# refresh-bio/vclust

Hardware: AMD Instinct MI355X
Metric: genome pairs/sec through prefilter+align (ani.tsv) (higher is better)
Workload: dtype u64

## Files before the change

include/vclust_gpu.h:

```cpp
#ifndef VCLUST_GPU_H
#define VCLUST_GPU_H

#include <stdint.h>

#ifdef __cplusplus
extern "C" {
#endif

enum {
    VG_OK = 0, VG_EINVAL = -1, VG_EIO = -2, VG_ENODEV = -3, VG_EHIP = -4, VG_ENOMEM = -5,
    VG_EOVERFLOW = -6
};

const char* vg_version(void);
const char* vg_last_error(void);
void        vg_free(void* p);
int vg_device_count(void);
int vg_set_device(int device);
void vg_release_device_memory(void);
int vg_alloc_selftest(const int64_t* sizes, int n_sizes, int cycles);
int vg_copy(void* dst, const void* src, int64_t bytes, int to_host);

typedef struct vg_genomes vg_genomes;

// ... 4 lines not shown
int vg_genomes_from_codes(const uint8_t* codes, const int64_t* offsets, int n_genomes,
                          const char* const* names, vg_genomes** out);
void        vg_genomes_free(vg_genomes* g);
int         vg_genomes_count(const vg_genomes* g);
int64_t     vg_genomes_total_len(const vg_genomes* g);
int         vg_genomes_lengths(const vg_genomes* g, int64_t* out );
const char* vg_genomes_name(const vg_genomes* g, int idx);
int         vg_genomes_codes(const vg_genomes* g, int idx, uint8_t* out);
int vg_genomes_to_device(vg_genomes* g);

typedef struct { uint32_t a, b, shared; } vg_pair_count;

int vg_kmer_shared(vg_genomes* g, int k, double fraction, int shard, int n_shards,
                   uint32_t min_shared, int64_t* set_sizes, vg_pair_count** pairs,
                   int64_t* n_pairs);
int vg_kmer_shared_new(vg_genomes* g, int n_db, int k, double fraction, uint32_t min_shared, int64_t* set_sizes,
                       vg_pair_count** pairs, int64_t* n_pairs);
void vg_set_new_path(int mode);
typedef struct {
    int accepted; int64_t P; int n_passes;
    int levels, total_bits, B1, B2;
    int st_tiles; int64_t n_st; int u_st, g_st;
    int tile32k, narrow, short_rec;
} vg_kmer_geometry_info;
int vg_kmer_geometry(const vg_genomes* g, int k, double fraction, int shard, int n_shards, vg_kmer_geometry_info* info);
int vg_kmer_geometry_at(int64_t padded_positions, int k, vg_kmer_geometry_info* info);
int vg_kmer_set(vg_genomes* g, int idx, int k, double fraction, uint64_t** out, int64_t* n_out);

int vg_write_fltr(const vg_genomes* g, int k, double fraction, int min_kmers, double min_ident,
                  int max_seqs, const int64_t* set_sizes, const vg_pair_count* pairs,
                  int64_t n_pairs, const char* out_path);

int vg_filter_pairs(int k, int min_kmers, double min_ident, const int64_t* set_sizes, int64_t n_genomes,
                    const vg_pair_count* pairs, int64_t n_pairs, vg_pair_count** out, int64_t* n_out);

typedef struct {
    int    k;
    int    min_kmers;
    double min_ident;
    int    batch_size;
    double kmers_fraction;
    int    max_seqs;
    int    num_threads;
    int    verbosity;
    int    is_multifasta;
} vg_prefilter_params;
// ... 10 lines not shown
    uint32_t task; int32_t qstart, qend, rstart, rend; int32_t n_match;
} vg_region;

typedef struct { int weak_seed_ratio, anchor_margin, seed_choice; } vg_lz_fit;
void vg_set_lz_fit(const vg_lz_fit* f);

int vg_lz_align(vg_genomes* g, const vg_task* tasks, int64_t n_tasks, const vg_lz_params* p,
                vg_pair_stat* stats, vg_region** regions, int64_t* n_regions);

int vg_lz_prepare(vg_genomes* g, const vg_pair_count* pairs, int64_t n_pairs, const vg_lz_params* p);

int vg_align_order(const vg_genomes* g, int32_t* order );
int vg_read_filter(const vg_genomes* g, const char* path, double thr,
                   vg_pair_count** pairs, int64_t* n_pairs);

int vg_align_tasks(const vg_genomes* g, const vg_pair_count* pairs, int64_t n_pairs,
                   vg_task** tasks, int64_t* n_tasks);
int vg_lz_index_dump(vg_genomes* g, int idx, const vg_lz_params* p,
                     uint32_t** bucket_end, uint32_t** entries, int64_t* n_entries,
                     int* pos_bits, int* tag_bits, int* path);
void vg_set_index_budget(int64_t bytes);
void vg_set_subshards(int n);
void vg_set_range_scan(int mode);
void vg_set_placement_trials(int n);

typedef struct {
    vg_lz_params lz;
    double out_tani, out_gani, out_ani, out_qcov, out_rcov;
    const char* filter_path; double filter_threshold;
    const char* out_aln_path;
    const char* const* out_columns; int n_out_columns;
    int num_threads; int verbosity; int is_multifasta;
} vg_align_params;
int vg_write_ani(const vg_genomes* g, const vg_task* tasks, const vg_pair_stat* stats,
                 int64_t n_tasks, const vg_region* regions, int64_t n_regions,
                 const char* out_path, const vg_align_params* p);
int vg_align(const char* const* fasta_paths, int n_paths, const char* out_path,
             const vg_align_params* p);

int vg_align_new(const char* const* db_paths, int n_db_paths, const char* const* new_paths, int n_new_paths,
                 const char* out_path, const vg_align_params* p);

typedef struct vg_comm vg_comm;
typedef int (*vg_allgather_fn)(void* ctx, const void* send, void* recv, int64_t bytes, int on_device);
int  vg_comm_create(int rank, int world, vg_allgather_fn allgather, void* ctx, vg_comm** out);
int  vg_rccl_unique_id(void* out , int64_t bytes);
// ... 134 lines not shown
```

vclust_amd/_lib.py:

```python
import ctypes as C
import pathlib

PKG_DIR = pathlib.Path(__file__).resolve().parent
LIB_PATH = PKG_DIR / 'libvclust_gpu.so'


class VclustGpuError(RuntimeError):
    def __init__(self, code, msg):
        super().__init__(f'libvclust_gpu error {code}: {msg}')
        self.code = code


class PairCount(C.Structure):
    _fields_ = [('a', C.c_uint32), ('b', C.c_uint32), ('shared', C.c_uint32)]


class Task(C.Structure):
    _fields_ = [('q', C.c_uint32), ('r', C.c_uint32)]


class PairStat(C.Structure):
    _fields_ = [('n_match', C.c_uint32), ('aln_len', C.c_uint32), ('n_regions', C.c_uint32)]


# ... 53 lines not shown
class DedupStats(C.Structure):
    _fields_ = [('records', C.c_int64), ('unique', C.c_int64), ('removed', C.c_int64), ('reverse', C.c_int64),
                ('rounds', C.c_int64), ('collisions', C.c_int64)]


class DedupOptions(C.Structure):
    _fields_ = [('circular', C.c_int)]


class DedupContainedStats(C.Structure):
    _fields_ = [('passes', C.c_int64), ('positions', C.c_int64), ('hits', C.c_int64), ('candidates', C.c_int64),
                ('verified', C.c_int64), ('slices', C.c_int64)]


class DedupRepeatStats(C.Structure):
    _fields_ = [('with_repeat', C.c_int64), ('repeat_symbols', C.c_int64), ('candidates', C.c_int64), ('equal', C.c_int64),
                ('batches', C.c_int64)]


class KmerGeometry(C.Structure):
    _fields_ = [('accepted', C.c_int), ('P', C.c_int64), ('n_passes', C.c_int),
                ('levels', C.c_int), ('total_bits', C.c_int), ('B1', C.c_int), ('B2', C.c_int),
                ('st_tiles', C.c_int), ('n_st', C.c_int64), ('u_st', C.c_int), ('g_st', C.c_int),
                ('tile32k', C.c_int), ('narrow', C.c_int), ('short_rec', C.c_int)]


class KernelTime(C.Structure):
    _fields_ = [('name', C.c_char * 48), ('total_ms', C.c_double), ('launches', C.c_int64),
                ('bytes', C.c_double)]


ALLGATHER_FN = C.CFUNCTYPE(C.c_int, C.c_void_p, C.c_void_p, C.c_void_p, C.c_int64, C.c_int)

P = C.POINTER
SYMBOLS = {
    'vg_version': (C.c_char_p, []),
    'vg_last_error': (C.c_char_p, []),
    'vg_free': (None, [C.c_void_p]),
    'vg_device_count': (C.c_int, []),
    'vg_set_device': (C.c_int, [C.c_int]),
    'vg_release_device_memory': (None, []),
    'vg_copy': (C.c_int, [C.c_void_p, C.c_void_p, C.c_int64, C.c_int]),
    'vg_alloc_selftest': (C.c_int, [C.POINTER(C.c_int64), C.c_int, C.c_int]),
    'vg_genomes_load': (C.c_int, [P(C.c_char_p), C.c_int, C.c_int, C.c_int, P(C.c_void_p)]),
    'vg_genomes_load_db_new': (C.c_int, [P(C.c_char_p), C.c_int, P(C.c_char_p), C.c_int, C.c_int, C.c_int, P(C.c_void_p), P(C.c_int)]),
    'vg_genomes_from_codes': (C.c_int, [C.c_void_p, C.c_void_p, C.c_int, P(C.c_char_p), P(C.c_void_p)]),
    'vg_genomes_free': (None, [C.c_void_p]),
# ... 8 lines not shown
    'vg_kmer_shared_new': (C.c_int, [C.c_void_p, C.c_int, C.c_int, C.c_double, C.c_uint32, P(C.c_int64), P(P(PairCount)), P(C.c_int64)]),
    'vg_kmer_geometry': (C.c_int, [C.c_void_p, C.c_int, C.c_double, C.c_int, C.c_int, P(KmerGeometry)]),
    'vg_kmer_geometry_at': (C.c_int, [C.c_int64, C.c_int, P(KmerGeometry)]),
    'vg_kmer_set': (C.c_int, [C.c_void_p, C.c_int, C.c_int, C.c_double, P(P(C.c_uint64)), P(C.c_int64)]),
    'vg_filter_pairs': (C.c_int, [C.c_int, C.c_int, C.c_double, C.POINTER(C.c_int64), C.c_int64, C.POINTER(PairCount), C.c_int64,
                                  C.POINTER(C.POINTER(PairCount)), C.POINTER(C.c_int64)]),
    'vg_write_fltr': (C.c_int, [C.c_void_p, C.c_int, C.c_double, C.c_int, C.c_double, C.c_int,
                                P(C.c_int64), P(PairCount), C.c_int64, C.c_char_p]),
    'vg_prefilter': (C.c_int, [P(C.c_char_p), C.c_int, C.c_char_p, P(PrefilterParams)]),
    'vg_prefilter_new': (C.c_int, [P(C.c_char_p), C.c_int, P(C.c_char_p), C.c_int, C.c_char_p, P(PrefilterParams)]),
    'vg_set_process_ends_after_call': (None, [C.c_int]),
    'vg_set_lz_fit': (None, [P(LzFit)]),
    'vg_lz_align': (C.c_int, [C.c_void_p, P(Task), C.c_int64, P(LzParams), P(PairStat),
                              P(P(Region)), P(C.c_int64)]),
    'vg_align_order': (C.c_int, [C.c_void_p, P(C.c_int32)]),
    'vg_read_filter': (C.c_int, [C.c_void_p, C.c_char_p, C.c_double, P(P(PairCount)), P(C.c_int64)]),
    'vg_align_tasks': (C.c_int, [C.c_void_p, P(PairCount), C.c_int64, P(P(Task)), P(C.c_int64)]),
    'vg_lz_prepare': (C.c_int, [C.c_void_p, P(PairCount), C.c_int64, P(LzParams)]),
    'vg_lz_index_dump': (C.c_int, [C.c_void_p, C.c_int, P(LzParams), P(P(C.c_uint32)), P(P(C.c_uint32)), P(C.c_int64),
                                   P(C.c_int), P(C.c_int), P(C.c_int)]),
    'vg_set_index_budget': (None, [C.c_int64]),
    'vg_set_subshards': (None, [C.c_int]),
    'vg_set_range_scan': (None, [C.c_int]),
    'vg_set_new_path': (None, [C.c_int]),
    'vg_set_placement_trials': (None, [C.c_int]),
    'vg_write_ani': (C.c_int, [C.c_void_p, P(Task), P(PairStat), C.c_int64, P(Region), C.c_int64,
                               C.c_char_p, P(AlignParams)]),
    'vg_align': (C.c_int, [P(C.c_char_p), C.c_int, C.c_char_p, P(AlignParams)]),
    'vg_align_new': (C.c_int, [P(C.c_char_p), C.c_int, P(C.c_char_p), C.c_int, C.c_char_p, P(AlignParams)]),
    'vg_comm_create': (C.c_int, [C.c_int, C.c_int, C.c_void_p, C.c_void_p, P(C.c_void_p)]),
    'vg_rccl_unique_id': (C.c_int, [C.c_void_p, C.c_int64]),
    'vg_comm_rccl_create': (C.c_int, [C.c_int, C.c_int, C.c_void_p, C.c_int64, P(C.c_void_p)]),
    'vg_comm_free': (None, [C.c_void_p]),
    'vg_comm_kind': (C.c_int, [C.c_void_p]),
    'vg_comm_rccl_ranks': (C.c_int, [C.c_void_p]),
    'vg_comm_rank': (C.c_int, [C.c_void_p]),
    'vg_comm_world': (C.c_int, [C.c_void_p]),
    'vg_comm_selftest': (C.c_int, [C.c_void_p, C.c_int64]),
    'vg_kmer_shared_sharded': (C.c_int, [C.c_void_p, C.c_int, C.c_double, C.c_uint32, C.c_void_p, P(C.c_int64), P(P(PairCount)), P(C.c_int64)]),
    'vg_align_owner': (C.c_int, [P(Task), C.c_int64, C.c_int, C.c_int, P(C.c_int32)]),
    'vg_align_pairs_share': (C.c_int, [C.c_void_p, P(PairCount), C.c_int64, C.c_int, C.c_int, P(P(Task)), P(C.c_int64)]),
    'vg_lz_align_pairs_sharded': (C.c_int, [C.c_void_p, P(PairCount), C.c_int64, P(LzParams), C.c_void_p, P(P(Task)), P(C.c_int64), P(P(PairStat))]),
    'vg_lz_align_sharded': (C.c_int, [C.c_void_p, P(Task), C.c_int64, P(LzParams), C.c_void_p, P(PairStat), P(P(Region)), P(C.c_int64)]),
    'vg_prefilter_sharded': (C.c_int, [P(C.c_char_p), C.c_int, C.c_char_p, P(PrefilterParams), C.c_void_p]),
    'vg_align_sharded': (C.c_int, [P(C.c_char_p), C.c_int, C.c_char_p, P(AlignParams), C.c_void_p]),
    'vg_cluster': (C.c_int, [C.c_char_p, C.c_char_p, C.c_char_p, P(ClusterParams)]),
# ... 70 lines not shown
```

vclust_amd/api.py:

```python
import ctypes as C
import inspect
import os

import numpy as np

from . import _lib
from ._lib import (CLUSTER_ALGORITHMS, LINKAGE_ALGORITHMS, AlignParams, ClusterStats, DedupStats, KernelTime, LinkageStats, LzParams, PairCount, PairStat,
                   PrefilterParams, Region, Task, check)

ALIGN_FIELDS = ['qidx', 'ridx', 'query', 'reference', 'tani', 'gani', 'ani', 'qcov', 'rcov',
                'num_alns', 'len_ratio', 'qlen', 'rlen', 'nt_match', 'nt_mismatch']

PAIR_DTYPE = np.dtype([('a', '<u4'), ('b', '<u4'), ('shared', '<u4')])
TASK_DTYPE = np.dtype([('q', '<u4'), ('r', '<u4')])
STAT_DTYPE = np.dtype([('n_match', '<u4'), ('aln_len', '<u4'), ('n_regions', '<u4')])
REGION_DTYPE = np.dtype([('task', '<u4'), ('qstart', '<i4'), ('qend', '<i4'), ('rstart', '<i4'),
                         ('rend', '<i4'), ('n_match', '<i4')])
LINKAGE_DTYPE = np.dtype([('node_a', '<i8'), ('node_b', '<i8'), ('similarity', '<f8'), ('size', '<i8'), ('object_a', '<i4'),
                          ('object_b', '<i4')])

from .stages import DEFAULT_LZ


def version():
# ... 396 lines not shown


def dedup_set_hash_bits(bits=128):
    _lib.load().vg_dedup_set_hash_bits(int(bits))


def dedup_set_anchor_symbols(w=16):
    _lib.load().vg_dedup_set_anchor_symbols(int(w))


def dedup_set_index_positions(n=0):
    _lib.load().vg_dedup_set_index_positions(int(n))


def set_lz_fit(weak_seed_ratio=3, anchor_margin=-1, seed_choice=3):
    f = _lib.LzFit(int(weak_seed_ratio), int(anchor_margin), int(seed_choice))
    _lib.load().vg_set_lz_fit(C.byref(f))


def set_range_scan(mode):
    _lib.load().vg_set_range_scan(int(mode))


def set_placement_trials(n):
    _lib.load().vg_set_placement_trials(int(n))


def set_new_path(mode):
    _lib.load().vg_set_new_path(int(mode))


def kmer_geometry_at(padded_positions, k=25):
    info = _lib.KmerGeometry()
    check(_lib.load().vg_kmer_geometry_at(int(padded_positions), int(k), C.byref(info)))
    return {name: int(getattr(info, name)) for name, _ in info._fields_}


def release_device_memory():
    _lib.load().vg_release_device_memory()


def profile_enable(on=True):
    _lib.load().vg_profile_enable(int(bool(on)))


def profile_reset():
# ... 10 lines not shown
```

vclust_amd/csrc/vg_prefilter.hip:

```cpp
#include "vg_common.h"
#include <functional>
#include <map>
#include <mutex>
#include <optional>
#include <rocprim/rocprim.hpp>
#include <algorithm>
#include <cmath>
#include <cstring>

namespace {

constexpr uint64_t SENT = ~0ULL;
constexpr uint32_t SCRAMBLE32 = 0x9E3779B1u;
__host__ __device__ __forceinline__ uint64_t scramble_key(uint64_t cano, int k) {
    const uint32_t L = (uint32_t)cano & ((1u << k) - 1u);
    const uint32_t H = (uint32_t)(cano >> k);
    return ((uint64_t)(H ^ ((L * SCRAMBLE32) >> (32 - k))) << k) | L;
}
__host__ __device__ __forceinline__ uint64_t unscramble_key(uint64_t key, int k) { return scramble_key(key, k); }
constexpr uint32_t DUP_BIT = 0x80000000u;

__device__ __forceinline__ uint64_t mix64(uint64_t x) {
    x ^= x >> 33; x *= 0xff51afd7ed558ccdULL; x ^= x >> 33;
    x *= 0xc4ceb9fe1a85ec53ULL; x ^= x >> 33; return x;
// ... 1255 lines not shown
                }
                lds_sync();
                for (uint32_t slot = threadIdx.x; slot < n_sub; slot += PT_THREADS) {
                    const uint32_t i = s_perm[slot];
                    const uint64_t key = kmer_key_lds(S.A, s_pk, s_list[i]);
                    uint32_t v[3];
                    key_words(key, S.k2, &v[0], &v[1]);
                    v[2] = row0 + i;
                    const uint32_t b = B1 ? (v[0] >> (32 - B1)) - (uint32_t)S.bin_lo : 0u;
                    const uint64_t dst = (uint64_t)cursor[b] + (slot - tstart[b]);
                    if (short_kr > 0) {
                        const uint64_t r = ((key & ((1ULL << short_kr) - 1)) << SR_POS_BITS) | (uint64_t)((v[2] - grp_row0) & ((1u << SR_POS_BITS) - 1u));
                        __builtin_memcpy(o_rec + 2 * dst, &r, 8);
                    } else __builtin_memcpy(o_rec + 3 * dst, v, 12);
                }
                lds_sync();
                for (int b = threadIdx.x; b < nbins; b += PT_THREADS) cursor[b] += thist[b];
                lds_sync();
            }
        }
    }
}

constexpr int NT_TILE = 16384;
constexpr int NT_PER = NT_TILE / PT_THREADS;
constexpr int NT_MAXBINS = 2048;
template <bool SHORT>
__global__ void __launch_bounds__(PT_THREADS)
k_part_scatter2_narrow(const uint32_t* __restrict__ rec, int B1, int B2, int64_t n_units, const uint32_t* __restrict__ Ts, lvl2_tab L,
                       uint32_t* __restrict__ o_rec, int narrow_shift) {
    __shared__ uint2 s_rec[NT_TILE];
    __shared__ uint32_t thist[NT_MAXBINS], tstart[NT_MAXBINS], cursor[NT_MAXBINS];
    __shared__ uint32_t s_wave[16];
    const int nbins = 1 << B2;
    const int lane = threadIdx.x & 63, wv = threadIdx.x >> 6;
    for (int64_t u = blockIdx.x; u < n_units; u += gridDim.x) {
        uint32_t b1, U; int64_t s0, s1;
        lvl2_unit(L, u, &b1, &U, &s0, &s1);
        uint32_t gbase = 0, gb[3] = {0, 0, 0};
        uint32_t grow0 = 0, grow1 = 0, grow2 = 0, grow3 = 0;
        if (SHORT) {
            lvl2_groups(L, b1, U, s1, &gbase, gb);
            if (L.wbase) {
                const int64_t w0 = (int64_t)(gbase >> 6), gw = 1LL << (SR_POS_BITS - 6);
                grow0 = L.wbase[min(w0, L.W)]; grow1 = L.wbase[min(w0 + gw, L.W)]; grow2 = L.wbase[min(w0 + 2 * gw, L.W)]; grow3 = L.wbase[min(w0 + 3 * gw, L.W)];
            }
        }
        lds_sync();
        for (int b = threadIdx.x; b < nbins; b += PT_THREADS) cursor[b] = Ts[((uint64_t)b1 * L.n_u + U) * nbins + b];
        for (int64_t t0 = s0; t0 < s1; t0 += NT_TILE) {
            for (int b = threadIdx.x; b < nbins; b += PT_THREADS) thist[b] = 0;
            lds_sync();
            uint32_t key[NT_PER], pay[NT_PER], br[NT_PER];
            if (SHORT) {
                uint4 rr[NT_PER / 2];
#pragma unroll
                for (int p = 0; p < NT_PER / 2; ++p) {
                    const int64_t i = t0 + 2 * ((int64_t)p * PT_THREADS + threadIdx.x);
                    rr[p] = make_uint4(0u, 0u, 0u, 0u);
                    if (i + 1 < s1) __builtin_memcpy(&rr[p], rec + 2 * i, 16);
                    else if (i < s1) __builtin_memcpy(&rr[p].x, rec + 2 * i, 8);
                }
#pragma unroll
                for (int p = 0; p < NT_PER / 2; ++p) {
#pragma unroll
                    for (int h = 0; h < 2; ++h) {
                        const int j = 2 * p + h;
                        const int64_t i = t0 + 2 * ((int64_t)p * PT_THREADS + threadIdx.x) + h;
                        br[j] = 0xffffffffu; key[j] = 0; pay[j] = 0;
                        if (i < s1) {
                            const uint64_t r = h ? (((uint64_t)rr[p].w << 32) | rr[p].z) : (((uint64_t)rr[p].y << 32) | rr[p].x);
                            const uint32_t ui = (uint32_t)i;
                            const uint32_t gsel = (uint32_t)(ui >= gb[0]) + (uint32_t)(ui >= gb[1]) + (uint32_t)(ui >= gb[2]);
                            key[j] = (uint32_t)(r >> SR_POS_BITS) << (32 - (L.kr - B2));
                            const uint32_t low = (uint32_t)r & ((1u << SR_POS_BITS) - 1u);
                            pay[j] = L.wbase ? (gsel == 0 ? grow0 : gsel == 1 ? grow1 : gsel == 2 ? grow2 : grow3) + low : gbase + (gsel << SR_POS_BITS) + low;
                            br[j] = (uint32_t)(r >> (SR_POS_BITS + L.kr - B2)) & (uint32_t)(nbins - 1);
                        }
                    }
                }
            } else {
#pragma unroll
                for (int j = 0; j < NT_PER; ++j) {
                    const int64_t i = t0 + (int64_t)j * PT_THREADS + threadIdx.x;
                    br[j] = 0xffffffffu; key[j] = 0; pay[j] = 0;
                    if (i < s1) {
                        uint32_t r[3]; __builtin_memcpy(r, rec + 3 * i, 12);
                        key[j] = (uint32_t)(((((uint64_t)r[0] << 32) | r[1]) << narrow_shift) >> 32); pay[j] = r[2];
                        br[j] = (r[0] >> (32 - B1 - B2)) & (uint32_t)(nbins - 1);
                    }
                }
            }
#pragma unroll
            for (int j = 0; j < NT_PER; ++j) if (br[j] != 0xffffffffu) br[j] |= atomicAdd(&thist[br[j]], 1u) << 11;
            lds_sync();
            {
                constexpr int BPT = NT_MAXBINS / PT_THREADS;
                uint32_t cn[BPT], tot = 0;
#pragma unroll
                for (int v = 0; v < BPT; ++v) { const int b = BPT * (int)threadIdx.x + v; cn[v] = b < nbins ? thist[b] : 0u; tot += cn[v]; }
                uint32_t run = block_scan_1024(tot, s_wave, nullptr);
#pragma unroll
                for (int v = 0; v < BPT; ++v) { const int b = BPT * (int)threadIdx.x + v; if (b < nbins) tstart[b] = run; run += cn[v]; }
            }
            lds_sync();
#pragma unroll
            for (int j = 0; j < NT_PER; ++j) if (br[j] != 0xffffffffu) s_rec[tstart[br[j] & 0x7ffu] + (br[j] >> 11)] = make_uint2(key[j], pay[j]);
            lds_sync();
            const int per_wave = (nbins + 15) >> 4;
            for (int bb = wv * per_wave; bb < min(nbins, (wv + 1) * per_wave); bb += 8) {
                const int b = bb + (lane >> 3);
                const bool live = b < min(nbins, (wv + 1) * per_wave);
                const uint32_t st = live ? tstart[b] : 0u, cnt = live ? thist[b] : 0u;
                const uint64_t cur = live ? cursor[b] : 0ull;
                for (uint32_t i = (uint32_t)(lane & 7); __any(i < cnt); i += 8) {
                    if (i < cnt) { const uint2 v = s_rec[st + i]; __builtin_memcpy(o_rec + 2 * (cur + i), &v, 8); }
                }
            }
            lds_sync();
            for (int b = threadIdx.x; b < nbins; b += PT_THREADS) cursor[b] += thist[b];
            lds_sync();
        }
    }
}

constexpr int SC_SLAB = 128;
__global__ void __launch_bounds__(PT_THREADS)
k_scan_columns_a(const uint32_t* __restrict__ T, int64_t n_rows, int n_cols, uint32_t* __restrict__ S) {
    const int64_t r0 = (int64_t)blockIdx.x * SC_SLAB, r1 = min(n_rows, r0 + SC_SLAB);
    for (int c = threadIdx.x; c < n_cols; c += PT_THREADS) {
        uint32_t sum = 0;
        for (int64_t r = r0; r < r1; ++r) sum += T[r * n_cols + c];
        S[(int64_t)blockIdx.x * n_cols + c] = sum;
    }
}
__global__ void __launch_bounds__(PT_THREADS)
k_scan_columns_b(uint32_t* __restrict__ S, int n_slabs, int n_cols , uint32_t* __restrict__ start ) {
    __shared__ uint32_t s_wave[16];
    constexpr int CPT = PT_MAXBINS / PT_THREADS;
// ... 611 lines not shown
    } else {
        std::vector<int64_t> m_roff((size_t)W + 1), t_roff((size_t)W + 1);
        for (int r = 0; r <= W; ++r) { m_roff[(size_t)r] = word_of(r) * 8; t_roff[(size_t)r] = st_of(r) * (int64_t)nb1 * 4; }
        if (mine.m_off.empty()) { mine.m_off.assign((size_t)W + 1, 0); mine.t_off.assign((size_t)W + 1, 0); }
        if (status != VG_OK) vg_set_error("%s", err.c_str());
        const vg_xpart parts[2] = { { mine.mask.p, mine.m_off.data(), wave_mask, m_roff.data() }, { mine.T.p, mine.t_off.data(), T1s, t_roff.data() } };
        xs->alltoallv(status, parts, 2);
    }
    if (W_total > 0) hipLaunchKernelGGL(k_mask_popc, dim3(grid_for(W_total)), dim3(256), 0, s, (const unsigned long long*)wave_mask, W_total, wave_cnt);
    VG_HIP(hipStreamSynchronize(s));
}

struct kmer_index {
    sorted_index si;
    dbuf<uint32_t> arena;
    dbuf<uint32_t> rowinfo, gen; dbuf<int> d_dups;
    std::vector<int> kept, dups;
    int64_t nv = 0, n_rows_info = 0;
    bool compact_rows = false, rows_from_map = false;
    const uint32_t* wbase = nullptr;
};
struct bucket_geometry {
    bool range, big_buckets, narrow, tile32k, short_rec;
    int total_bits, B1, B2, levels, bin_lo, nb1g, nb1, nb2, st_tiles, n_slabs; int64_t n_st, nbk;
    lvl2_tab L2;
};
static bool bucket_geometry_for(int k, bool dense, const kmer_args& A, int64_t n_src, bucket_geometry& G) {
    G.range = dense && A.dig_n < (1u << DIG_BITS);
    if (g_sw.radix || n_src < (1 << 16) || n_src >= (1LL << 32)) return false;
    const int64_t n_expect = dense && !G.range ? n_src / std::max<uint32_t>(1u, A.n_shards) : n_src;
    if (!bucket_digits(n_expect, &G.total_bits, &G.B1, &G.B2)) return false;
    G.big_buckets = (n_expect >> G.total_bits) > 1024; G.levels = G.total_bits > 11 ? 2 : 1;
    if (G.range && G.B1 > DIG_BITS) return false;
    G.bin_lo = G.range ? (int)(A.dig_lo >> (DIG_BITS - G.B1)) : 0;
    G.nb1g = 1 << G.B1; G.nb2 = 1 << G.B2;
    G.nb1 = G.range ? (int)(((A.dig_lo + A.dig_n - 1) >> (DIG_BITS - G.B1)) - (uint32_t)G.bin_lo + 1) : G.nb1g;
    G.nbk = G.levels == 1 ? G.nb1 : (int64_t)G.nb1 * G.nb2;
    G.narrow = G.levels == 2 && 2 * k - G.total_bits <= 32;
    G.st_tiles = (int)std::max<int64_t>(1, std::min<int64_t>(dense ? 16 : 8, n_src / ((int64_t)PT_TILE * 2048)));
    if (dense && G.st_tiles >= 4) G.st_tiles &= ~3;
    const int64_t st_pos = (int64_t)G.st_tiles * PT_TILE;
    G.n_st = (n_src + st_pos - 1) / st_pos; G.n_slabs = (int)((G.n_st + SC_SLAB - 1) / SC_SLAB);
    lvl2_tab& L2 = G.L2; memset(&L2, 0, sizeof L2);
    L2.n_st = G.n_st; L2.nb1 = G.nb1; L2.kr = 2 * k - G.B1;
    L2.u_st = (int)std::max<int64_t>(1, std::min<int64_t>(G.n_st, (65536LL * G.nb1g) / st_pos)); L2.n_u = (int)((G.n_st + L2.u_st - 1) / L2.u_st);
    { int sh = 0; while ((1LL << sh) < st_pos) ++sh; L2.st_shift = sh; }
    G.tile32k = dense && G.st_tiles % 4 == 0 && G.B1 <= 12 && !g_sw.old_scatter;
    G.short_rec = G.levels == 2 && G.tile32k && G.narrow && G.B2 <= 11 && L2.kr + SR_POS_BITS <= 64 && L2.kr - G.B2 >= 1 &&
                  (st_pos & (st_pos - 1)) == 0 && st_pos <= (1LL << SR_POS_BITS) && !g_sw.long_rec;
    if (G.short_rec) {
        const int64_t g_st = (1LL << SR_POS_BITS) / st_pos;
        if (L2.u_st <= g_st) L2.g_st = (g_st % L2.u_st == 0) ? 0 : -1;
        else L2.g_st = (L2.u_st % g_st == 0 && L2.u_st / g_st <= 4) ? (int)g_st : -1;
        if (L2.g_st < 0) { G.short_rec = false; L2.g_st = 0; }
    }
    return true;
}
struct bucket_run {
    vg_genomes* g; int k; bool dense; const pass_inputs& in; kmer_index& ix; int* d_kept; hipStream_t s;
    bucket_geometry G; part_src S; compact_map cmap;
    bool k25 = false; uint32_t n1 = 0; size_t n_cap = 0;
    const uint32_t* f_rec = nullptr; int f_stride = 3;
    dbuf<uint32_t> T1s, slab, d_off1, a_rec, b_rec;
    struct ev_guard { hipEvent_t e = nullptr; hipStream_t st; ~ev_guard() { if (e) { (void)hipStreamWaitEvent(st, e, 0); (void)hipEventDestroy(e); } } } rows_zero;
    dbuf<uint32_t> boff;
};
struct level1_tmp { std::optional<vg_prof_scope> ps; dbuf<uint32_t> wave_cnt; dbuf<char> scan_tmp; };
static void clear_rows_aside(bucket_run& R) {
    if (!(R.G.levels == 2 && R.dense && !R.G.range)) return;
    dbuf<uint32_t>& rowinfo = R.ix.rowinfo; const int64_t n_rows_info = R.ix.n_rows_info; hipEvent_t& ev_rows_zero = R.rows_zero.e;
    static const size_t tot = [] { size_t fr0 = 0, t0 = 0; return hipMemGetInfo(&fr0, &t0) == hipSuccess ? t0 : (size_t)0; }();
    if (tot && (size_t)n_rows_info * 4 * 8 <= tot / 2) try {
        { vg_dev_try_scope opportunistic; rowinfo.alloc((size_t)n_rows_info); }
        hipStream_t side = vg_side_stream();
        hipEvent_t ev_s = nullptr;
        VG_HIP(hipEventCreateWithFlags(&ev_s, hipEventDisableTiming));
        VG_HIP(hipEventRecord(ev_s, R.s));
        VG_HIP(hipStreamWaitEvent(side, ev_s, 0));
// ... 68 lines not shown
    if (G.tile32k && G.range && G.nb1 <= RG_MAXBINS && !g_sw.range_dense) {
        const bool kc = R.k == 25 && !A.use_frac;
        if (tile64k) with_k(kc, [&](auto K) { hipLaunchKernelGGL((k_part_scatter_range<K(), 65536>), dim3(grid_s), dim3(PT_THREADS), 0, s, S, G.B1, G.nb1, G.st_tiles / 8, G.n_st, T1s, a_rec, tsh); });
        else with_k(kc, [&](auto K) { hipLaunchKernelGGL((k_part_scatter_range<K(), 32768>), dim3(grid_s), dim3(PT_THREADS), 0, s, S, G.B1, G.nb1, G.st_tiles / 4, G.n_st, T1s, a_rec, tsh); });
    }
    else if (G.tile32k) with_k(R.k25 && !G.range, [&](auto K) { hipLaunchKernelGGL(k_part_scatter_dense<K()>, dim3(grid_s), dim3(PT_THREADS), 0, s, S, G.B1, G.nb1, G.st_tiles / 4, G.n_st, T1s, a_rec, tsh); });
    else if (R.dense) hipLaunchKernelGGL((k_part_scatter<SRC_DENSE, 1>), dim3(grid_s), dim3(PT_THREADS), 0, s, S, G.B1, 0, G.st_tiles, G.n_st, T1s, lvl2_tab{}, a_rec, -1, G.nb1);
    else hipLaunchKernelGGL((k_part_scatter<SRC_ARRAYS, 1>), dim3(grid_s), dim3(PT_THREADS), 0, s, S, G.B1, 0, G.st_tiles, G.n_st, T1s, lvl2_tab{}, a_rec, -1, G.nb1);
}
static void level2(bucket_run& R) {
    const bucket_geometry& G = R.G; const lvl2_tab& L2 = G.L2; hipStream_t s = R.s; kmer_index& ix = R.ix;
    const int64_t n_units = (int64_t)G.nb1 * L2.n_u;
    const size_t t2n = (size_t)G.nb1 * (size_t)G.nb2 * (size_t)L2.n_u;
    dbuf<uint32_t> T2s(t2n);
    const uint32_t* a_rec = R.a_rec.p;
    {
        vg_prof_scope ps("kmer_partition2", (double)R.n1 * (4.0 + (G.short_rec ? 8.0 : 12.0) + (G.narrow ? 8.0 : 12.0)));
        const int grid_c2 = (int)std::min<int64_t>(n_units, 512);
        hipLaunchKernelGGL(G.short_rec ? k_part_count2<true> : k_part_count2<false>, dim3(grid_c2), dim3(PT_THREADS), 0, s, a_rec, G.B1, G.B2, n_units, L2, T2s.p);
        hipLaunchKernelGGL(k_scan_units, dim3(G.nb1), dim3(PT_THREADS), 0, s, T2s.p, L2.n_u, G.nb2, (const uint32_t*)R.d_off1.p, G.nb1, R.boff.p);
        R.b_rec.alloc((G.narrow ? 2 : 3) * R.n_cap + 8);
        const int grid_s2 = (int)std::min<int64_t>(n_units, 256);
        if (G.short_rec || (G.narrow && G.B2 <= 11 && !g_sw.staged2))
            hipLaunchKernelGGL(G.short_rec ? k_part_scatter2_narrow<true> : k_part_scatter2_narrow<false>, dim3(grid_s2), dim3(PT_THREADS), 0, s, a_rec, G.B1, G.B2, n_units,
                               (const uint32_t*)T2s.p, L2, R.b_rec.p, G.total_bits);
        else {
            part_src S2; memset(&S2, 0, sizeof S2);
            S2.rec = a_rec; S2.n = (int64_t)R.n1; S2.k2 = 2 * R.k;
            hipLaunchKernelGGL((k_part_scatter<SRC_PLANES, 2>), dim3(grid_s2), dim3(PT_THREADS), 0, s, S2, G.B1, G.B2, 0, n_units,
                               (const uint32_t*)T2s.p, L2, R.b_rec.p, G.narrow ? G.total_bits : -1, 0);
        }
    }
    VG_HIP(hipStreamSynchronize(s));
    vg_host_mark("buckets: level 2 done");
    vg_deferred_start();
    R.f_rec = R.b_rec.p; R.f_stride = G.narrow ? 2 : 3;
    ix.arena = std::move(R.a_rec);
    if (!R.rows_zero.e) ix.rowinfo.view(ix.arena.p, (size_t)ix.n_rows_info);
    ix.gen.view(ix.arena.p + (((size_t)ix.n_rows_info + 3) & ~(size_t)3), (size_t)R.n1 + 4);
}
static void bucket_kernels(bucket_run& R) {
    const bucket_geometry& G = R.G; hipStream_t s = R.s; vg_genomes* g = R.g; kmer_index& ix = R.ix;
    const uint32_t n1 = R.n1; const int64_t nbk = G.nbk;
    if (ix.gen.n < (size_t)n1 + 4) ix.gen.alloc((size_t)n1 + 4);
    if (ix.rowinfo.n < (size_t)ix.n_rows_info) ix.rowinfo.alloc((size_t)ix.n_rows_info);
    dbuf<unsigned int> d_nover(2); d_nover.zero(s);
    dbuf<uint32_t> over1((size_t)nbk), over2;
    if (R.rows_zero.e) VG_HIP(hipStreamWaitEvent(s, R.rows_zero.e, 0));
// ... 610 lines not shown
                           int64_t* set_sizes, dbuf<vg_pair_count>& pairs, int64_t* n_pairs, vg_slice_exchange* xs, int* mode_out) {
    if (mode_out) *mode_out = 0;
    vg_require_device();
    int rc = vg_genomes_to_device(g); if (rc) throw vg_error(rc, vg_last_error());
    *n_pairs = 0;
    if (g->n == 0) return;
    const shard_plan plan = plan_shards(g, fraction, n_shards, false);
    if (mode_out) *mode_out = plan.range ? 1 : 2;
    unsigned long long n = 0; int sub = plan.sub;
    if (plan.one_pass) {
        std::vector<vg_pair_count> none; pass_inputs in; in.xs = xs;
        kmer_shared_pass(g, k, fraction, shard, n_shards, min_shared, set_sizes, none, in, &pairs, &n);
    } else for (int attempt = 0;; ++attempt) {
        try { kmer_shared_subshards(g, k, fraction, shard, n_shards, sub, min_shared, set_sizes, pairs, &n); break; }
        catch (const vg_error& e) { if (e.code != VG_EOVERFLOW || attempt >= 3 || !plan.retry_finer) throw; ++sub; pairs.release(); }
    }
    if (!plan.one_pass && !pairs.p) pairs.alloc(1);
    *n_pairs = (int64_t)n;
}

static_assert(sizeof(vg_pair_count) == 12, "pair record layout");
extern "C" void vg_set_subshards(int n) { g_force_subshards = n; }
extern "C" void vg_set_range_scan(int mode) { g_range_scan_mode = mode == 1 ? 1 : 0; }


static void report_geometry(int k, bool dense, const kmer_args& A, int64_t P, vg_kmer_geometry_info* info) {
    bucket_geometry G;
    info->accepted = dense ? (bucket_geometry_for(k, true, A, P, G) ? 1 : 0) : -1;
    if (info->accepted != 1) return;
    info->levels = G.levels; info->total_bits = G.total_bits; info->B1 = G.B1; info->B2 = G.B2;
    info->st_tiles = G.st_tiles; info->n_st = G.n_st; info->u_st = G.L2.u_st; info->g_st = G.L2.g_st;
    info->tile32k = G.tile32k; info->narrow = G.narrow; info->short_rec = G.short_rec;
}
extern "C" int vg_kmer_geometry(const vg_genomes* g, int k, double fraction, int shard, int n_shards, vg_kmer_geometry_info* info) {
    VG_API_BEGIN
    if (!g || !info) throw vg_error(VG_EINVAL, "vg_kmer_geometry: null argument");
    if (k < 8 || k > 31) throw vg_error(VG_EINVAL, "k out of range (8..31)");
    if (n_shards < 1 || shard < 0 || shard >= n_shards) throw vg_error(VG_EINVAL, "bad shard");
    if (!(fraction > 0.0) || fraction > 1.0) throw vg_error(VG_EINVAL, "fraction must be in (0,1]");
    memset(info, 0, sizeof *info);
    const int64_t P = g->padded_total();
    info->P = P; info->n_passes = 1;
    if (g->n == 0) return VG_OK;
    const shard_plan plan = plan_shards(g, fraction, n_shards, true);
    info->n_passes = plan.sub;
    const int sh = shard * plan.sub, ns = n_shards * plan.sub;
    const bool masked = subshards_share_scan(g, fraction, n_shards, plan.sub);
    const bool dense = pass_source_dense(P, fraction, ns, masked);
    report_geometry(k, dense, shard_kmer_args(P, g->align_shift, k, 1.0, sh, ns), P, info);
    VG_API_END
}
extern "C" int vg_kmer_geometry_at(int64_t padded_positions, int k, vg_kmer_geometry_info* info) {
    VG_API_BEGIN
    if (!info) throw vg_error(VG_EINVAL, "vg_kmer_geometry_at: null argument");
    if (k < 8 || k > 31) throw vg_error(VG_EINVAL, "k out of range (8..31)");
// ... 47 lines not shown
```

Baseline: 2.652 million.

## Process level-2 short-record scatter in 32K-record tiles with two LDS windows

Adds a templated tile size to the level-2 narrow partition scatter kernel. For short records with B2 >= 10 it histograms a 32K-record tile held in registers, storing each record's per-bin rank packed as 16 bits, then scatters and flushes it through the existing 16K-entry LDS buffer in two windows. The aim is to halve the per-tile histogram, scan and sync overhead and lengthen per-bin runs written to global memory. The cost is more registers per thread, a window-staged flush that re-walks bins, and a new setter and geometry field for choosing the tile.

```diff
diff --git a/include/vclust_gpu.h b/include/vclust_gpu.h
--- a/include/vclust_gpu.h
+++ b/include/vclust_gpu.h
@@ -50,6 +50,7 @@
     int levels, total_bits, B1, B2;
     int st_tiles; int64_t n_st; int u_st, g_st;
     int tile32k, narrow, short_rec;
+    int level2_tile;
 } vg_kmer_geometry_info;
 int vg_kmer_geometry(const vg_genomes* g, int k, double fraction, int shard, int n_shards, vg_kmer_geometry_info* info);
 int vg_kmer_geometry_at(int64_t padded_positions, int k, vg_kmer_geometry_info* info);
@@ -106,6 +107,7 @@
 void vg_set_index_budget(int64_t bytes);
 void vg_set_subshards(int n);
 void vg_set_range_scan(int mode);
+void vg_set_level2_tile(int records);
 void vg_set_placement_trials(int n);
 
 typedef struct {
diff --git a/vclust_amd/_lib.py b/vclust_amd/_lib.py
--- a/vclust_amd/_lib.py
+++ b/vclust_amd/_lib.py
@@ -99,7 +99,7 @@
     _fields_ = [('accepted', C.c_int), ('P', C.c_int64), ('n_passes', C.c_int),
                 ('levels', C.c_int), ('total_bits', C.c_int), ('B1', C.c_int), ('B2', C.c_int),
                 ('st_tiles', C.c_int), ('n_st', C.c_int64), ('u_st', C.c_int), ('g_st', C.c_int),
-                ('tile32k', C.c_int), ('narrow', C.c_int), ('short_rec', C.c_int)]
+                ('tile32k', C.c_int), ('narrow', C.c_int), ('short_rec', C.c_int), ('level2_tile', C.c_int)]
 
 
 class KernelTime(C.Structure):
@@ -154,6 +154,7 @@
     'vg_set_index_budget': (None, [C.c_int64]),
     'vg_set_subshards': (None, [C.c_int]),
     'vg_set_range_scan': (None, [C.c_int]),
+    'vg_set_level2_tile': (None, [C.c_int]),
     'vg_set_new_path': (None, [C.c_int]),
     'vg_set_placement_trials': (None, [C.c_int]),
     'vg_write_ani': (C.c_int, [C.c_void_p, P(Task), P(PairStat), C.c_int64, P(Region), C.c_int64,
diff --git a/vclust_amd/api.py b/vclust_amd/api.py
--- a/vclust_amd/api.py
+++ b/vclust_amd/api.py
@@ -442,6 +442,10 @@
     _lib.load().vg_set_range_scan(int(mode))
 
 
+def set_level2_tile(records=0):
+    _lib.load().vg_set_level2_tile(int(records))
+
+
 def set_placement_trials(n):
     _lib.load().vg_set_placement_trials(int(n))
 
diff --git a/vclust_amd/csrc/vg_prefilter.hip b/vclust_amd/csrc/vg_prefilter.hip
--- a/vclust_amd/csrc/vg_prefilter.hip
+++ b/vclust_amd/csrc/vg_prefilter.hip
@@ -1301,16 +1301,19 @@
     }
 }
 
-constexpr int NT_TILE = 16384;
-constexpr int NT_PER = NT_TILE / PT_THREADS;
+constexpr int NT_WIN = 16384;
 constexpr int NT_MAXBINS = 2048;
-template <bool SHORT>
+template <bool SHORT, int NT_TILE>
 __global__ void __launch_bounds__(PT_THREADS)
 k_part_scatter2_narrow(const uint32_t* __restrict__ rec, int B1, int B2, int64_t n_units, const uint32_t* __restrict__ Ts, lvl2_tab L,
                        uint32_t* __restrict__ o_rec, int narrow_shift) {
-    __shared__ uint2 s_rec[NT_TILE];
+    static_assert(NT_TILE == NT_WIN || (SHORT && NT_TILE == 2 * NT_WIN), "a tile is one window, or two of short records");
+    constexpr int NT_PER = NT_TILE / PT_THREADS;
+    constexpr bool WINDOWS = NT_TILE > NT_WIN;
+    __shared__ uint2 s_rec[NT_WIN];
     __shared__ uint32_t thist[NT_MAXBINS], tstart[NT_MAXBINS], cursor[NT_MAXBINS];
     __shared__ uint32_t s_wave[16];
+    __shared__ uint32_t s_sink[WINDOWS ? 64 : 1];
     const int nbins = 1 << B2;
     const int lane = threadIdx.x & 63, wv = threadIdx.x >> 6;
     for (int64_t u = blockIdx.x; u < n_units; u += gridDim.x) {
@@ -1325,75 +1328,159 @@
                 grow0 = L.wbase[min(w0, L.W)]; grow1 = L.wbase[min(w0 + gw, L.W)]; grow2 = L.wbase[min(w0 + 2 * gw, L.W)]; grow3 = L.wbase[min(w0 + 3 * gw, L.W)];
             }
         }
+        auto short_bin = [&](uint64_t r, int sh) { return (uint32_t)(r >> sh) & (uint32_t)(nbins - 1); };
+        const int bin_sh = SR_POS_BITS + L.kr - B2;
         lds_sync();
         for (int b = threadIdx.x; b < nbins; b += PT_THREADS) cursor[b] = Ts[((uint64_t)b1 * L.n_u + U) * nbins + b];
         for (int64_t t0 = s0; t0 < s1; t0 += NT_TILE) {
             for (int b = threadIdx.x; b < nbins; b += PT_THREADS) thist[b] = 0;
             lds_sync();
-            uint32_t key[NT_PER], pay[NT_PER], br[NT_PER];
-            if (SHORT) {
-                uint4 rr[NT_PER / 2];
+            uint4 rr[WINDOWS ? NT_PER / 2 : 1];
+            uint32_t rk[WINDOWS ? NT_PER / 2 : 1];
+            uint32_t key[WINDOWS ? 1 : NT_PER], pay[WINDOWS ? 1 : NT_PER], br[WINDOWS ? 1 : NT_PER];
+            int n_tile = 0;
+            if constexpr (WINDOWS) {
+                n_tile = (int)min((int64_t)NT_TILE, s1 - t0);
+                uint32_t l2 = 2u * threadIdx.x;
+                asm volatile("" : "+v"(l2));
+                const uint32_t* tp = rec + 2 * (t0 + l2);
 #pragma unroll
                 for (int p = 0; p < NT_PER / 2; ++p) {
-                    const int64_t i = t0 + 2 * ((int64_t)p * PT_THREADS + threadIdx.x);
                     rr[p] = make_uint4(0u, 0u, 0u, 0u);
-                    if (i + 1 < s1) __builtin_memcpy(&rr[p], rec + 2 * i, 16);
-                    else if (i < s1) __builtin_memcpy(&rr[p].x, rec + 2 * i, 8);
+                    if ((int)l2 + 1 < n_tile - 2 * PT_THREADS * p) __builtin_memcpy(&rr[p], tp + 4 * PT_THREADS * p, 16);
+                    else if ((int)l2 < n_tile - 2 * PT_THREADS * p) __builtin_memcpy(&rr[p].x, tp + 4 * PT_THREADS * p, 8);
                 }
-#pragma unroll
-                for (int p = 0; p < NT_PER / 2; ++p) {
-#pragma unroll
-                    for (int h = 0; h < 2; ++h) {
-                        const int j = 2 * p + h;
-                        const int64_t i = t0 + 2 * ((int64_t)p * PT_THREADS + threadIdx.x) + h;
+                uint32_t h2 = l2;
+                asm volatile("" : "+v"(h2));
+#pragma unroll
+                for (int g = 0; g < NT_PER / 8; ++g) {
+                    if (8 * PT_THREADS * g < n_tile) {
+#pragma unroll
+                        for (int p = 4 * g; p < 4 * g + 4; ++p) {
+                            const bool ok0 = (int)h2 < n_tile - 2 * PT_THREADS * p, ok1 = (int)h2 + 1 < n_tile - 2 * PT_THREADS * p;
+                            const uint32_t r0 = atomicAdd(ok0 ? &thist[short_bin(((uint64_t)rr[p].y << 32) | rr[p].x, bin_sh)] : &s_sink[lane], 1u);
+                            const uint32_t r1 = atomicAdd(ok1 ? &thist[short_bin(((uint64_t)rr[p].w << 32) | rr[p].z, bin_sh)] : &s_sink[lane], 1u);
+                            rk[p] = (ok0 ? r0 : 0xffffu) | ((ok1 ? r1 : 0xffffu) << 16);
+                        }
+                    } else {
+#pragma unroll
+                        for (int p = 4 * g; p < 4 * g + 4; ++p) rk[p] = 0xffffffffu;
+                    }
+                }
+            } else {
+                if (SHORT) {
+                    uint4 rr[NT_PER / 2];
+#pragma unroll
+                    for (int p = 0; p < NT_PER / 2; ++p) {
+                        const int64_t i = t0 + 2 * ((int64_t)p * PT_THREADS + threadIdx.x);
+                        rr[p] = make_uint4(0u, 0u, 0u, 0u);
+                        if (i + 1 < s1) __builtin_memcpy(&rr[p], rec + 2 * i, 16);
+                        else if (i < s1) __builtin_memcpy(&rr[p].x, rec + 2 * i, 8);
+                    }
+#pragma unroll
+                    for (int p = 0; p < NT_PER / 2; ++p) {
+#pragma unroll
+                        for (int h = 0; h < 2; ++h) {
+                            const int j = 2 * p + h;
+                            const int64_t i = t0 + 2 * ((int64_t)p * PT_THREADS + threadIdx.x) + h;
+                            br[j] = 0xffffffffu; key[j] = 0; pay[j] = 0;
+                            if (i < s1) {
+                                const uint64_t r = h ? (((uint64_t)rr[p].w << 32) | rr[p].z) : (((uint64_t)rr[p].y << 32) | rr[p].x);
+                                const uint32_t ui = (uint32_t)i;
+                                const uint32_t gsel = (uint32_t)(ui >= gb[0]) + (uint32_t)(ui >= gb[1]) + (uint32_t)(ui >= gb[2]);
+                                key[j] = (uint32_t)(r >> SR_POS_BITS) << (32 - (L.kr - B2));
+                                const uint32_t low = (uint32_t)r & ((1u << SR_POS_BITS) - 1u);
+                                pay[j] = L.wbase ? (gsel == 0 ? grow0 : gsel == 1 ? grow1 : gsel == 2 ? grow2 : grow3) + low : gbase + (gsel << SR_POS_BITS) + low;
+                                br[j] = (uint32_t)(r >> (SR_POS_BITS + L.kr - B2)) & (uint32_t)(nbins - 1);
+                            }
+                        }
+                    }
+                } else {
+#pragma unroll
+                    for (int j = 0; j < NT_PER; ++j) {
+                        const int64_t i = t0 + (int64_t)j * PT_THREADS + threadIdx.x;
                         br[j] = 0xffffffffu; key[j] = 0; pay[j] = 0;
                         if (i < s1) {
-                            const uint64_t r = h ? (((uint64_t)rr[p].w << 32) | rr[p].z) : (((uint64_t)rr[p].y << 32) | rr[p].x);
-                            const uint32_t ui = (uint32_t)i;
-                            const uint32_t gsel = (uint32_t)(ui >= gb[0]) + (uint32_t)(ui >= gb[1]) + (uint32_t)(ui >= gb[2]);
-                            key[j] = (uint32_t)(r >> SR_POS_BITS) << (32 - (L.kr - B2));
-                            const uint32_t low = (uint32_t)r & ((1u << SR_POS_BITS) - 1u);
-                            pay[j] = L.wbase ? (gsel == 0 ? grow0 : gsel == 1 ? grow1 : gsel == 2 ? grow2 : grow3) + low : gbase + (gsel << SR_POS_BITS) + low;
-                            br[j] = (uint32_t)(r >> (SR_POS_BITS + L.kr - B2)) & (uint32_t)(nbins - 1);
+                            uint32_t r[3]; __builtin_memcpy(r, rec + 3 * i, 12);
+                            key[j] = (uint32_t)(((((uint64_t)r[0] << 32) | r[1]) << narrow_shift) >> 32); pay[j] = r[2];
+                            br[j] = (r[0] >> (32 - B1 - B2)) & (uint32_t)(nbins - 1);
+                        }
+                    }
+                }
+#pragma unroll
+                for (int j = 0; j < NT_PER; ++j) if (br[j] != 0xffffffffu) br[j] |= atomicAdd(&thist[br[j]], 1u) << 11;
+            }
+            lds_sync();
+            {
+                constexpr int BPT = NT_MAXBINS / PT_THREADS;
+                uint32_t cn[BPT], tot = 0;
+#pragma unroll
+                for (int v = 0; v < BPT; ++v) { const int b = BPT * (int)threadIdx.x + v; cn[v] = b < nbins ? thist[b] : 0u; tot += cn[v]; }
+                uint32_t run = block_scan_1024(tot, s_wave, nullptr);
+#pragma unroll
+                for (int v = 0; v < BPT; ++v) { const int b = BPT * (int)threadIdx.x + v; if (b < nbins) tstart[b] = run; run += cn[v]; }
+            }
+            lds_sync();
+            if constexpr (WINDOWS) {
+                int gl[3];
+#pragma unroll
+                for (int j = 0; j < 3; ++j) gl[j] = __builtin_amdgcn_readfirstlane((int)max((int64_t)0, min((int64_t)NT_TILE, (int64_t)gb[j] - t0)));
+                for (uint32_t base = 0; base < (uint32_t)n_tile; base += NT_WIN) {
+                    if (base) lds_sync();
+                    uint32_t l2 = 2u * threadIdx.x;
+                    int sh = bin_sh, psh = SR_POS_BITS, ksh = 32 - (L.kr - B2), rsh = 16, g0 = gl[0], g1 = gl[1], g2 = gl[2];
+                    uint32_t pmask = (1u << SR_POS_BITS) - 1u, rmask = 0xffffu;
+                    asm volatile("" : "+v"(l2), "+s"(sh), "+s"(psh), "+s"(ksh), "+s"(rsh), "+s"(g0), "+s"(g1), "+s"(g2), "+s"(pmask), "+s"(rmask));
+#pragma unroll
+                    for (int g = 0; g < NT_PER / 8; ++g) {
+                        if (8 * PT_THREADS * g >= n_tile) break;
+                        uint32_t slot[8];
+#pragma unroll
+                        for (int q = 0; q < 8; ++q) {
+                            const int p = 4 * g + q / 2;
+                            const uint64_t r = q % 2 ? (((uint64_t)rr[p].w << 32) | rr[p].z) : (((uint64_t)rr[p].y << 32) | rr[p].x);
+                            slot[q] = tstart[short_bin(r, sh)] + ((q % 2 ? rk[p] >> rsh : rk[p]) & rmask) - base;
+                        }
+#pragma unroll
+                        for (int q = 0; q < 8; ++q) {
+                            if (slot[q] < (uint32_t)NT_WIN) {
+                                const int p = 4 * g + q / 2;
+                                const uint64_t r = q % 2 ? (((uint64_t)rr[p].w << 32) | rr[p].z) : (((uint64_t)rr[p].y << 32) | rr[p].x);
+                                const int c = 2 * PT_THREADS * p + q % 2;
+                                const uint32_t gsel = (uint32_t)((int)l2 >= g0 - c) + (uint32_t)((int)l2 >= g1 - c) + (uint32_t)((int)l2 >= g2 - c);
+                                const uint32_t low = (uint32_t)r & pmask;
+                                const uint32_t pay1 = L.wbase ? (gsel == 0 ? grow0 : gsel == 1 ? grow1 : gsel == 2 ? grow2 : grow3) + low : gbase + (gsel << SR_POS_BITS) + low;
+                                s_rec[slot[q]] = make_uint2((uint32_t)(r >> psh) << ksh, pay1);
+                            }
+                        }
+                    }
+                    lds_sync();
+                    const uint32_t w_end = base + NT_WIN;
+                    for (int bb = 4 * wv; bb < nbins; bb += 64) {
+                        const int b = bb + (lane >> 4);
+                        const bool live = b < nbins;
+                        const uint32_t st = live ? tstart[b] : 0u, cnt = live ? thist[b] : 0u;
+                        if (!__any(st < w_end)) break;
+                        const uint32_t lo = max(st, base), hi = min(st + cnt, w_end);
+                        const uint64_t cur = live ? cursor[b] : 0ull;
+                        for (uint32_t i = lo + (uint32_t)(lane & 15); __any(i < hi); i += 16) {
+                            if (i < hi) { const uint2 v = s_rec[i - base]; __builtin_memcpy(o_rec + 2 * (cur + (i - st)), &v, 8); }
                         }
                     }
                 }
             } else {
 #pragma unroll
-                for (int j = 0; j < NT_PER; ++j) {
-                    const int64_t i = t0 + (int64_t)j * PT_THREADS + threadIdx.x;
-                    br[j] = 0xffffffffu; key[j] = 0; pay[j] = 0;
-                    if (i < s1) {
-                        uint32_t r[3]; __builtin_memcpy(r, rec + 3 * i, 12);
-                        key[j] = (uint32_t)(((((uint64_t)r[0] << 32) | r[1]) << narrow_shift) >> 32); pay[j] = r[2];
-                        br[j] = (r[0] >> (32 - B1 - B2)) & (uint32_t)(nbins - 1);
+                for (int j = 0; j < NT_PER; ++j) if (br[j] != 0xffffffffu) s_rec[tstart[br[j] & 0x7ffu] + (br[j] >> 11)] = make_uint2(key[j], pay[j]);
+                lds_sync();
+                const int per_wave = (nbins + 15) >> 4;
+                for (int bb = wv * per_wave; bb < min(nbins, (wv + 1) * per_wave); bb += 8) {
+                    const int b = bb + (lane >> 3);
+                    const bool live = b < min(nbins, (wv + 1) * per_wave);
+                    const uint32_t st = live ? tstart[b] : 0u, cnt = live ? thist[b] : 0u;
+                    const uint64_t cur = live ? cursor[b] : 0ull;
+                    for (uint32_t i = (uint32_t)(lane & 7); __any(i < cnt); i += 8) {
+                        if (i < cnt) { const uint2 v = s_rec[st + i]; __builtin_memcpy(o_rec + 2 * (cur + i), &v, 8); }
                     }
-                }
-            }
-#pragma unroll
-            for (int j = 0; j < NT_PER; ++j) if (br[j] != 0xffffffffu) br[j] |= atomicAdd(&thist[br[j]], 1u) << 11;
-            lds_sync();
-            {
-                constexpr int BPT = NT_MAXBINS / PT_THREADS;
-                uint32_t cn[BPT], tot = 0;
-#pragma unroll
-                for (int v = 0; v < BPT; ++v) { const int b = BPT * (int)threadIdx.x + v; cn[v] = b < nbins ? thist[b] : 0u; tot += cn[v]; }
-                uint32_t run = block_scan_1024(tot, s_wave, nullptr);
-#pragma unroll
-                for (int v = 0; v < BPT; ++v) { const int b = BPT * (int)threadIdx.x + v; if (b < nbins) tstart[b] = run; run += cn[v]; }
-            }
-            lds_sync();
-#pragma unroll
-            for (int j = 0; j < NT_PER; ++j) if (br[j] != 0xffffffffu) s_rec[tstart[br[j] & 0x7ffu] + (br[j] >> 11)] = make_uint2(key[j], pay[j]);
-            lds_sync();
-            const int per_wave = (nbins + 15) >> 4;
-            for (int bb = wv * per_wave; bb < min(nbins, (wv + 1) * per_wave); bb += 8) {
-                const int b = bb + (lane >> 3);
-                const bool live = b < min(nbins, (wv + 1) * per_wave);
-                const uint32_t st = live ? tstart[b] : 0u, cnt = live ? thist[b] : 0u;
-                const uint64_t cur = live ? cursor[b] : 0ull;
-                for (uint32_t i = (uint32_t)(lane & 7); __any(i < cnt); i += 8) {
-                    if (i < cnt) { const uint2 v = s_rec[st + i]; __builtin_memcpy(o_rec + 2 * (cur + i), &v, 8); }
                 }
             }
             lds_sync();
@@ -2051,9 +2138,11 @@
 };
 struct bucket_geometry {
     bool range, big_buckets, narrow, tile32k, short_rec;
+    int level2_tile;
     int total_bits, B1, B2, levels, bin_lo, nb1g, nb1, nb2, st_tiles, n_slabs; int64_t n_st, nbk;
     lvl2_tab L2;
 };
+static int g_level2_tile = 0;
 static bool bucket_geometry_for(int k, bool dense, const kmer_args& A, int64_t n_src, bucket_geometry& G) {
     G.range = dense && A.dig_n < (1u << DIG_BITS);
     if (g_sw.radix || n_src < (1 << 16) || n_src >= (1LL << 32)) return false;
@@ -2083,6 +2172,7 @@
         else L2.g_st = (L2.u_st % g_st == 0 && L2.u_st / g_st <= 4) ? (int)g_st : -1;
         if (L2.g_st < 0) { G.short_rec = false; L2.g_st = 0; }
     }
+    G.level2_tile = G.levels != 2 ? 0 : !G.short_rec ? NT_WIN : g_level2_tile ? g_level2_tile : G.B2 >= 10 ? 2 * NT_WIN : NT_WIN;
     return true;
 }
 struct bucket_run {
@@ -2197,8 +2287,8 @@
         R.b_rec.alloc((G.narrow ? 2 : 3) * R.n_cap + 8);
         const int grid_s2 = (int)std::min<int64_t>(n_units, 256);
         if (G.short_rec || (G.narrow && G.B2 <= 11 && !g_sw.staged2))
-            hipLaunchKernelGGL(G.short_rec ? k_part_scatter2_narrow<true> : k_part_scatter2_narrow<false>, dim3(grid_s2), dim3(PT_THREADS), 0, s, a_rec, G.B1, G.B2, n_units,
-                               (const uint32_t*)T2s.p, L2, R.b_rec.p, G.total_bits);
+            hipLaunchKernelGGL((!G.short_rec ? k_part_scatter2_narrow<false, NT_WIN> : G.level2_tile == 2 * NT_WIN ? k_part_scatter2_narrow<true, 2 * NT_WIN> : k_part_scatter2_narrow<true, NT_WIN>),
+                               dim3(grid_s2), dim3(PT_THREADS), 0, s, a_rec, G.B1, G.B2, n_units, (const uint32_t*)T2s.p, L2, R.b_rec.p, G.total_bits);
         else {
             part_src S2; memset(&S2, 0, sizeof S2);
             S2.rec = a_rec; S2.n = (int64_t)R.n1; S2.k2 = 2 * R.k;
@@ -2855,6 +2945,7 @@
 static_assert(sizeof(vg_pair_count) == 12, "pair record layout");
 extern "C" void vg_set_subshards(int n) { g_force_subshards = n; }
 extern "C" void vg_set_range_scan(int mode) { g_range_scan_mode = mode == 1 ? 1 : 0; }
+extern "C" void vg_set_level2_tile(int records) { g_level2_tile = records == NT_WIN || records == 2 * NT_WIN ? records : 0; }
 
 
 static void report_geometry(int k, bool dense, const kmer_args& A, int64_t P, vg_kmer_geometry_info* info) {
@@ -2864,6 +2955,7 @@
     info->levels = G.levels; info->total_bits = G.total_bits; info->B1 = G.B1; info->B2 = G.B2;
     info->st_tiles = G.st_tiles; info->n_st = G.n_st; info->u_st = G.L2.u_st; info->g_st = G.L2.g_st;
     info->tile32k = G.tile32k; info->narrow = G.narrow; info->short_rec = G.short_rec;
+    info->level2_tile = G.level2_tile;
 }
 extern "C" int vg_kmer_geometry(const vg_genomes* g, int k, double fraction, int shard, int n_shards, vg_kmer_geometry_info* info) {
     VG_API_BEGIN
```

New measurement: 2.653 million, median of 6. No clear change (+0.1%).
